# nabw/poroelasticity-linear-solvers

Measured on AMD Instinct MI355X. Metric: Krylov iters/sec + SpMV achieved HBM GB/s, 3-field poroelastic 10M DoF, higher is better.
Workload: dtype f64

## Files before the change

include/pls.h:

```cpp
#ifndef PLS_H
#define PLS_H

#include <stdint.h>

#ifdef __cplusplus
extern "C" {
#endif

#define PLS_ABI_VERSION 1

typedef struct pls_csr {
    int64_t nrows;
    int64_t ncols;
    const int64_t *row_ptr;
    const int32_t *col;
    const double *val;
} pls_csr;

typedef struct pls_handle pls_handle;
typedef struct pls_comm pls_comm;

typedef int (*pls_allgather_fn)(const void *send, int64_t bytes, void *recv, void *user);

typedef struct pls_result {
// ... 89 lines not shown
                              double *c_val);
int pls_hessenberg_eigenvalues(int m, const double *H, int ldh, double *re, double *im);

int pls_export_matrix(pls_handle *h, int which, int64_t *nrows, int64_t *nnz,
                      int64_t *row_ptr, int32_t *col, double *val);
int pls_get_permutation(pls_handle *h, int64_t *perm);

int pls_boomeramg_host_level(const pls_csr *A, const char *options, const char *prefix, int64_t level,
                             int64_t *nlevels, int64_t *n, int64_t *nc, int64_t *p_nnz, int8_t *cf, int64_t *p_rp,
                             int32_t *p_ci, double *p_v);

int pls_sparse_lu_analyze(const pls_csr *A, const char *options, double *stats, int64_t nstats, int32_t *perm,
                          int32_t *front_of, int32_t *parent);

typedef struct pls_anderson pls_anderson;
int pls_anderson_create(int32_t order, int64_t n, pls_anderson **out);
int pls_anderson_next(pls_anderson *a, double *d_gk);
int pls_anderson_destroy(pls_anderson *a);

int pls_bench_spmv(pls_handle *h, const double *d_x, double *d_y, int32_t reps, double *sec_per_launch);
int pls_bench_spmv_single(pls_handle *h, const double *d_x, double *d_y, int32_t reps, double *sec_per_launch);
int pls_spmv_layout(pls_handle *h, int32_t *d16, int64_t *matrix_bytes);
int pls_spmv_layout_single(pls_handle *h, int32_t *d16, int64_t *matrix_bytes);
int pls_bench_copy(int64_t bytes, int32_t reps, int32_t read_only, double *gbs);

#ifdef __cplusplus
}
#endif
#endif
```

poroelasticity-linear-solvers_amd/csrc/capi.cpp:

```cpp
#include <hip/hip_runtime.h>

#include <algorithm>
#include <atomic>
#include <chrono>
#include <numeric>

#include "../../include/pls.h"
#include "runtime.hpp"
#include "amg_host.hpp"
#include "anderson.hpp"
#include "bccols.hpp"
#include "blockpc.hpp"
#include "dist.hpp"
#include "synthetic.hpp"

namespace pls {

static thread_local std::string g_last_error;

static std::string checked_pc_type(const Options &o) {
    std::string pt = o.str("pls.pc_type", "diagonal");
    std::replace(pt.begin(), pt.end(), '_', ' ');
    static const char *ok[] = {"undrained", "undrained 3-way", "diagonal", "diagonal 3-way", "diagonal 3-way-II", "lu"};
    for (auto s : ok)
// ... 21 lines not shown
    std::unique_ptr<KSP> outer;
    AAR aar;
    DBuf<double> vout;
    pls_result res{};
    std::vector<double> history;
    std::unique_ptr<MatOp> Aop;
    Coupling coupling;
    bool coupling_stale = true;

    void parse_params() {
        pc_type = checked_pc_type(opt);
        three_way = (pc_type == "diagonal 3-way" || pc_type == "undrained 3-way");
        solver_type = opt.str("pls.solver_type", "gmres");
        inner_ksp = opt.str("pls.inner_ksp_type", "gmres");
        inner_pc = opt.str("pls.inner_pc_type", "hypre");
        timers.enabled = opt.flag("pls.timers", true);
        ctx.sell_d16 = opt.flag("pls.sell_d16", true);
        ctx.d16_wide_lpr = (int)opt.integer("pls.d16_wide_lpr", 8);
        if (ctx.d16_wide_lpr != 1 && ctx.d16_wide_lpr != 2 && ctx.d16_wide_lpr != 4 && ctx.d16_wide_lpr != 8 &&
            ctx.d16_wide_lpr != 16 && ctx.d16_wide_lpr != 32 && ctx.d16_wide_lpr != 64)
            throw Error("pls.d16_wide_lpr must be a power of two <= 64");
        ctx.d16_unroll = (int)opt.integer("pls.d16_unroll", 4);
        ctx.d16_xcd = (int)opt.integer("pls.d16_xcd", 0);
        ctx.d16_unroll_single = (int)opt.integer("pls.d16_unroll_single", 8);
        if (ctx.d16_unroll_single != 1 && ctx.d16_unroll_single != 2 && ctx.d16_unroll_single != 4 &&
            ctx.d16_unroll_single != 8)
            throw Error("pls.d16_unroll_single must be 1, 2, 4 or 8");
        ctx.halo_overlap = opt.flag("pls.halo_overlap", true);
        ctx.d16_segs = (int)opt.integer("pls.d16_segs", D16_SEG);
        if (ctx.d16_segs != D16_SEG && ctx.d16_segs != D16_SEG_MAX) throw Error("pls.d16_segs must be 4 or 8");
        ctx.d16_sigma = (int)opt.integer("pls.d16_sigma", 1024);
        if (ctx.d16_sigma < 0 || ctx.d16_sigma % 64) throw Error("pls.d16_sigma must be a multiple of 64 (0: off)");
        ctx.d16_sigma_pad = opt.num("pls.d16_sigma_pad", 0.15);
        ctx.d16_sorted_lpr = (int)opt.integer("pls.d16_sorted_lpr", 2);
        ctx.spmv_b3 = opt.flag("pls.spmv_b3", false);
        ctx.spmv_rcm = (int)opt.integer("pls.spmv_rcm", -1);
        ctx.sweep_chain = (int)opt.integer("pls.sweep_chain", -1);
        ctx.sweep_window = (int)opt.integer("pls.sweep_window", -1);
        ctx.ilu_factor_dep = (int)opt.integer("pls.ilu_factor_dep", 1);
        ctx.ilu_view = (int)opt.integer("pls.ilu_view", 0);
        ctx.ilu0_stage_cap = (int)opt.integer("pls.ilu0_stage", -1);
        ctx.ilu_dep_grid = (int)opt.integer("pls.ilu_dep_grid", 0);
        ctx.window_depth = (int)opt.integer("pls.window_depth", 2);
        if (ctx.window_depth != 2 && ctx.window_depth != 3) throw Error("pls.window_depth must be 2 or 3");
        ctx.window_ring = (int)opt.integer("pls.window_ring", -1);
        ctx.window_mixed = (int)opt.integer("pls.window_mixed", -1);
// ... 922 lines not shown
        (void)hipStreamDestroy(st);
    })
}

int pls_spmv_layout(pls_handle *hh, int32_t *d16, int64_t *matrix_bytes) {
    PLS_TRY({
        Handle &H = *reinterpret_cast<Handle *>(hh);
        build_sell(H.A, H.ctx);
        if (d16) *d16 = H.A.sell && H.A.sell->d16 ? 1 : 0;
        if (matrix_bytes) *matrix_bytes = H.A.sell ? H.A.sell->bytes() : 0;
    })
}

int pls_spmv_layout_single(pls_handle *hh, int32_t *d16, int64_t *matrix_bytes) {
    PLS_TRY({
        Handle &H = *reinterpret_cast<Handle *>(hh);
        build_sell(H.A, H.ctx);
        const bool ok = H.A.sell && H.A.sell->d16 && !H.A.sell->b3_nslices;
        if (d16) *d16 = ok ? 1 : 0;
        if (matrix_bytes) *matrix_bytes = ok ? H.A.sell->bytes_low() : 0;
    })
}

}
```

poroelasticity-linear-solvers_amd/csrc/kernels.hip:

```cpp
#include "devutil.hpp"

#include <hipcub/hipcub.hpp>

#include <type_traits>

namespace pls {

__device__ __forceinline__ double wave_reduce(double v) {
#pragma unroll
    for (int o = 32; o > 0; o >>= 1) v += __shfl_xor(v, o);
    return v;
}

#pragma clang fp contract(off)

__device__ __forceinline__ uint64_t mix64(uint64_t z) {
    z += 0x9E3779B97F4A7C15ULL;
    z = (z ^ (z >> 30)) * 0xBF58476D1CE4E5B9ULL;
    z = (z ^ (z >> 27)) * 0x94D049BB133111EBULL;
    return z ^ (z >> 31);
}
__device__ __forceinline__ uint64_t hash3(uint64_t s, uint64_t a, uint64_t b) {
    return mix64(mix64(mix64(s) ^ a) ^ b);
}
// ... 1526 lines not shown
    int32_t last = 0;
    for (int64_t k = 0; k < L; ++k) {
        const int64_t j = k * lpr + sub;
        uint16_t d = 0;
        double v = 0.0;
        if (j < len) {
            const int32_t c = ci[s0 + j];
            v = val[s0 + j];
            const int64_t gap = (int64_t)c - (int64_t)last;
            if (k == 0 || gap > 65535 || gap <= 0) {
                seg[slot * nsegs + nseg++] = c;
            } else {
                d = (uint16_t)gap;
            }
            last = c;
        }
        dl[base + (k >> 3) * 512 + lane * 8 + (k & 7)] = d;
        dv[base + (k >> 1) * 128 + lane * 2 + (k & 1)] = v;
    }
    if (nseg == 0) seg[slot * nsegs + nseg++] = 0;
    for (int j = nseg; j < nsegs; ++j) seg[slot * nsegs + j] = seg[slot * nsegs + nseg - 1];
}

__global__ __launch_bounds__(TPB) void k_first_col(int64_t nrows, const int64_t *rp, const int32_t *ci, int32_t *c0) {
    const int64_t r = (int64_t)blockIdx.x * TPB + threadIdx.x;
    if (r < nrows) c0[r] = rp[r + 1] > rp[r] ? ci[rp[r]] : -1;
}

typedef int32_t d16_i4 __attribute__((ext_vector_type(4)));
typedef uint32_t d16_u4 __attribute__((ext_vector_type(4)));
typedef double d16_d2 __attribute__((ext_vector_type(2)));
typedef float d16_f4 __attribute__((ext_vector_type(4)));

template <class V>
struct d16_values;
template <>
struct d16_values<double> {
    typedef d16_d2 pack;
    static constexpr int PER = 2, UNROLL_MAX = 4;
    static constexpr bool AUX_STORE = true;
    static __device__ __forceinline__ double get(const pack v, int e) { return e ? v.y : v.x; }
};
template <>
struct d16_values<float> {
    typedef d16_f4 pack;
    static constexpr int PER = 4, UNROLL_MAX = 8;
    static constexpr bool AUX_STORE = false;
    static __device__ __forceinline__ double get(const pack v, int e) {
        return (double)(e == 0 ? v.x : e == 1 ? v.y : e == 2 ? v.z : v.w);
    }
};

template <int G2, int TAG, bool HALO, int SEG, int AUX, class V>
__global__ __launch_bounds__(TPB) void k_d16_spmv(int64_t nrows, int64_t nslices, const int64_t *__restrict__ sptr,
                                                  const int64_t *__restrict__ sfirst,
                                                  const int32_t *__restrict__ slpr,
                                                  const uint16_t *__restrict__ dl, const V *__restrict__ dv,
                                                  const int32_t *__restrict__ seg, const double *__restrict__ x,
                                                  double *__restrict__ y, double alpha, double beta,
                                                  const double *__restrict__ z, const double *__restrict__ ghost,
                                                  int32_t nlocal, const int32_t *__restrict__ slist,
                                                  const int32_t *__restrict__ rowmap, double *aux, int d16_xcd) {
    static_assert(SEG == 4 || SEG == 8, "segment bases are one or two int4 per lane");
    static_assert(AUX != D16_AUX_STORE || d16_values<V>::AUX_STORE, "the raw-sum store belongs to the fp64 launch");
    typedef typename d16_values<V>::pack pack;
    constexpr int PER = d16_values<V>::PER, NQ = 8 / PER;
    const int lane = threadIdx.x & 63;
    unsigned blk = blockIdx.x;
    if (d16_xcd) {
        const unsigned per = (gridDim.x + 7) / 8;
        blk = (blockIdx.x % 8) * per + blockIdx.x / 8;
    }
    const int64_t idx = __builtin_amdgcn_readfirstlane((int)(blk * (TPB / 64) + (threadIdx.x >> 6)));
    if (idx >= nslices) return;
    const int64_t sl = slist ? (int64_t)__builtin_amdgcn_readfirstlane(slist[idx]) : idx;
    const int64_t base = sptr[sl];
    const int64_t L = (sptr[sl + 1] - base) >> 6;
    const int lpr = slpr[sl];
    const int64_t r0 = sfirst[sl], r1 = sfirst[sl + 1];
    const int64_t row = r0 + lane / lpr;
    const d16_i4 sb = __builtin_nontemporal_load(reinterpret_cast<const d16_i4 *>(seg) + (sl * 64 + lane) * (SEG / 4));
    d16_i4 sb2 = sb;
    if (SEG == 8) sb2 = __builtin_nontemporal_load(reinterpret_cast<const d16_i4 *>(seg) + (sl * 64 + lane) * 2 + 1);
    const d16_u4 *dp = reinterpret_cast<const d16_u4 *>(dl + base) + lane;
    const pack *vp = reinterpret_cast<const pack *>(dv + base) + lane;
    int32_t col = 0;
    int si = 0;
    double acc = 0.0;
    if (AUX == D16_AUX_INIT && lpr == 1 && row < r1) acc = aux[row];
    const int64_t ng = L >> 3;
    for (int64_t g0 = 0; g0 < ng; g0 += G2) {
        d16_u4 d[G2];
        pack v[G2][NQ];
#pragma unroll
        for (int u = 0; u < G2; ++u) {
            const int64_t g = g0 + u < ng ? g0 + u : ng - 1;
            d[u] = __builtin_nontemporal_load(dp + g * 64);
#pragma unroll
            for (int q = 0; q < NQ; ++q) v[u][q] = __builtin_nontemporal_load(vp + (g * NQ + q) * 64);
        }
#pragma unroll
        for (int u = 0; u < G2; ++u) {
            if (g0 + u >= ng) break;
            const uint32_t w[4] = {d[u].x, d[u].y, d[u].z, d[u].w};
#pragma unroll
            for (int e = 0; e < 8; ++e) {
                const int32_t dd = (int32_t)((w[e >> 1] >> ((e & 1) * 16)) & 0xffffu);
                int32_t b = si == 0 ? sb.x : si == 1 ? sb.y : si == 2 ? sb.z : sb.w;
                if (SEG == 8 && si >= 4) b = si == 4 ? sb2.x : si == 5 ? sb2.y : si == 6 ? sb2.z : sb2.w;
                col = dd == 0 ? b : col + dd;
                si += dd == 0 ? 1 : 0;
                const double a = d16_values<V>::get(v[u][e / PER], e % PER);
                if (HALO) {
                    const bool loc = col < nlocal;
                    const double xv = loc ? x[(uint32_t)col] : ghost[(uint32_t)(col - nlocal)];
                    acc += a * xv;
                } else {
                    acc += a * x[(uint32_t)col];
                }
            }
// ... 11 lines not shown
        y[yr] = r;
    }
}

void launch_d16_slice_len(int64_t nslices, const int64_t *sfirst, const int32_t *slpr, const int64_t *rp,
                          int64_t nrows, int64_t *slen, hipStream_t st, const int32_t *rowmap, const int64_t *rstart) {
    k_d16_slice_len<<<grid_for((nslices + 1) * 64, TPB), TPB, 0, st>>>(nslices, sfirst, slpr, rp, nrows, slen, rowmap,
                                                                       rstart);
}
void launch_d16_count(int64_t nslices, const int64_t *sfirst, const int32_t *slpr, const int64_t *rp,
                      const int32_t *ci, int64_t nrows, int32_t *maxseg, hipStream_t st, const int32_t *rowmap,
                      const int64_t *rstart) {
    if (nslices > 0)
        k_d16_count<<<grid_for(nslices * 64, TPB), TPB, 0, st>>>(nslices, sfirst, slpr, rp, ci, nrows, maxseg, rowmap,
                                                                 rstart);
}
void launch_d16_fill(int64_t nslices, const int64_t *sfirst, const int32_t *slpr, const int64_t *rp,
                     const int32_t *ci, const double *val, int64_t nrows, const int64_t *sptr, uint16_t *dl,
                     double *dv, int32_t *seg, int nsegs, hipStream_t st, const int32_t *rowmap,
                     const int64_t *rstart) {
    if (nslices > 0)
        k_d16_fill<<<grid_for(nslices * 64, TPB), TPB, 0, st>>>(nslices, sfirst, slpr, rp, ci, val, nrows, sptr, dl,
                                                                dv, seg, nsegs, rowmap, rstart);
}
__global__ __launch_bounds__(TPB) void k_coupling_rows(int64_t n, int64_t ns, const int64_t *rp, const int32_t *ci,
                                                       const double *val, const int64_t *mrp, const int32_t *mci,
                                                       const double *mval, const uint8_t *reuse, int64_t *rstart,
                                                       int32_t *differs) {
    const int64_t r = (int64_t)blockIdx.x * TPB + threadIdx.x;
    if (r >= n) return;
    const int64_t s = rp[r], e = rp[r + 1];
    if (r < ns) {
        rstart[r] = s;
        return;
    }
    int64_t lo = s, hi = e;
    while (lo < hi) {
        const int64_t mid = (lo + hi) >> 1;
        if (ci[mid] < ns) lo = mid + 1;
        else hi = mid;
    }
    const int64_t m0 = mrp[r - ns], cnt = lo - s;
    bool same = mrp[r - ns + 1] - m0 == cnt;
    for (int64_t k = 0; k < cnt && same; ++k)
        same = ci[s + k] == mci[m0 + k] && __double_as_longlong(val[s + k]) == __double_as_longlong(mval[m0 + k]);
    if (!same) *differs = 1;
// ... 9 lines not shown
    if (nrows > 0) k_first_col<<<grid_for(nrows, TPB), TPB, 0, st>>>(nrows, rp, ci, c0);
}
template <class V>
struct D16Call {
    unsigned g;
    size_t shm;
    hipStream_t st;
    int64_t nrows, ns;
    D16Streams L;
    const V *dv;
    const double *x;
    double *y;
    double alpha, beta;
    const double *z, *ghost;
    int32_t nl;
    const int32_t *slist, *rm;
    double *aux;
    int d16_xcd;
};
template <int G2, int TAG, bool HALO, int SEG, int AUX, class V>
static void d16_go(const D16Call<V> &a) {
    k_d16_spmv<G2, TAG, HALO, SEG, AUX, V><<<a.g, TPB, a.shm, a.st>>>(a.nrows, a.ns, a.L.sptr, a.L.sfirst, a.L.slpr,
                                                                      a.L.dl, a.dv, a.L.seg, a.x, a.y, a.alpha, a.beta,
                                                                      a.z, a.ghost, a.nl, a.slist, a.rm, a.aux, a.d16_xcd);
}
template <int G2, int SEG, class V>
static void d16_dispatch(const D16Call<V> &a, int tag, int aux_mode) {
    if constexpr (d16_values<V>::AUX_STORE)
        if (aux_mode == D16_AUX_STORE) return d16_go<G2, 0, false, SEG, D16_AUX_STORE>(a);
    if (aux_mode != D16_AUX_NONE) return d16_go<G2, 1, false, SEG, D16_AUX_INIT>(a);
    if (a.ghost) {
        if (tag) d16_go<G2, 1, true, SEG, D16_AUX_NONE>(a);
        else d16_go<G2, 0, true, SEG, D16_AUX_NONE>(a);
    } else {
        if (tag) d16_go<G2, 1, false, SEG, D16_AUX_NONE>(a);
        else d16_go<G2, 0, false, SEG, D16_AUX_NONE>(a);
    }
}
template <int SEG, class V>
static void d16_unrolled(int unroll, const D16Call<V> &a, int tag, int aux_mode) {
    switch (unroll) {
        case 1: d16_dispatch<1, SEG>(a, tag, aux_mode); break;
        case 2: d16_dispatch<2, SEG>(a, tag, aux_mode); break;
        case 4: d16_dispatch<4, SEG>(a, tag, aux_mode); break;
        default: d16_dispatch<d16_values<V>::UNROLL_MAX, SEG>(a, tag, aux_mode); break;
    }
}
// ... 865 lines not shown
```

poroelasticity-linear-solvers_amd/csrc/kernels.hpp:

```cpp
#pragma once
#include <hip/hip_runtime.h>
#include <cstdint>

namespace pls {

struct SynthDev {
    int32_t dim;
    uint64_t seed;
    double delta;
    int64_t n[3];
    int64_t off[3];
    int32_t cnt[6];
    const int32_t *offs[6];
    int64_t rlo[3], rlen[3], rloff[3], nrows;
};
void launch_synth_count(const SynthDev &S, int64_t *row_len, hipStream_t st);
void launch_synth_fill(const SynthDev &S, int variant, const int64_t *row_ptr, int32_t *col,
                       double *val, hipStream_t st);
void launch_synth_rhs(const SynthDev &S, uint64_t seed, double *b, hipStream_t st);

void exclusive_scan_i64(const int64_t *in, int64_t *out, int64_t n, void *tmp, size_t tmp_bytes,
                        hipStream_t st);
size_t exclusive_scan_tmp_bytes(int64_t n);

// ... 146 lines not shown
void launch_iluk_scatter(int64_t n, const int64_t *srp, const int32_t *sci, const double *sval, const int64_t *drp,
                         const int32_t *dci, double *dval, int32_t *fail, hipStream_t st);

int64_t sell_nslices(int64_t nrows);
void launch_sell_slice_len(int64_t nrows, const int64_t *rp, int64_t *slen , hipStream_t st);
void launch_sell_fill(int64_t nrows, const int64_t *rp, const int32_t *ci, const double *val, const int64_t *sptr,
                      int32_t *scol, double *sval, hipStream_t st);
void launch_sell_spmv(int64_t nrows, const int64_t *sptr, const int32_t *scol, const double *sval, const double *x,
                      double *y, double alpha, double beta, const double *z, int tag, const double *ghost,
                      int64_t nlocal, hipStream_t st);
constexpr int D16_SEG = 4;
constexpr int D16_SEG_MAX = 8;
void launch_d16_slice_len(int64_t nslices, const int64_t *sfirst, const int32_t *slpr, const int64_t *rp,
                          int64_t nrows, int64_t *slen , hipStream_t st,
                          const int32_t *rowmap = nullptr ,
                          const int64_t *rstart = nullptr);
void launch_d16_count(int64_t nslices, const int64_t *sfirst, const int32_t *slpr, const int64_t *rp,
                      const int32_t *ci, int64_t nrows, int32_t *maxseg, hipStream_t st,
                      const int32_t *rowmap = nullptr, const int64_t *rstart = nullptr);
void launch_d16_fill(int64_t nslices, const int64_t *sfirst, const int32_t *slpr, const int64_t *rp,
                     const int32_t *ci, const double *val, int64_t nrows, const int64_t *sptr, uint16_t *dl,
                     double *dv, int32_t *seg, int nsegs , hipStream_t st,
                     const int32_t *rowmap = nullptr, const int64_t *rstart = nullptr);
void launch_coupling_rows(int64_t n, int64_t ns, const int64_t *rp, const int32_t *ci, const double *val,
                          const int64_t *mrp, const int32_t *mci, const double *mval, const uint8_t *reuse,
                          int64_t *rstart, int32_t *differs, hipStream_t st);
constexpr int D16_AUX_NONE = 0, D16_AUX_STORE = 1, D16_AUX_INIT = 2;
void launch_first_col(int64_t nrows, const int64_t *rp, const int32_t *ci, int32_t *c0, hipStream_t st);
struct D16Streams {
    const int64_t *sptr, *sfirst;
    const int32_t *slpr;
    const uint16_t *dl;
    const int32_t *seg;
    int nsegs;
};
void launch_d16_spmv(int64_t nrows, int64_t nslices, const D16Streams &L, const double *dv, const double *x, double *y,
                     double alpha, double beta, const double *z, int tag, const double *ghost, int64_t nlocal,
                     int unroll ,
                     int d16_xcd ,
                     hipStream_t st,
                     const int32_t *slist = nullptr ,
                     const int32_t *rowmap = nullptr ,
                     size_t lds_reserve = 0 ,
                     int aux_mode = D16_AUX_NONE, double *aux = nullptr );
void launch_d16_round_values(int64_t stored, const double *dv, float *dv32, int32_t *overflow, hipStream_t st);
void launch_d16_spmv(int64_t nrows, int64_t nslices, const D16Streams &L, const float *dv32, const double *x, double *y,
                     double alpha, double beta, const double *z, int tag, const double *ghost, int64_t nlocal,
                     int unroll, int d16_xcd, hipStream_t st, const int32_t *slist = nullptr,
                     const int32_t *rowmap = nullptr, size_t lds_reserve = 0, const double *aux_init = nullptr);
void launch_triple_flags(int64_t n, const int64_t *rp, const int32_t *ci, uint8_t *flag, hipStream_t st);
int b3_lanes_per_triple();
void launch_b3_fill(int64_t nslices, int64_t ntrip, const int64_t *bptr, const int32_t *tmap, const int64_t *rp,
                    const int32_t *ci, const double *val, int32_t *bcol, double *bval, hipStream_t st);
void launch_b3_spmv(int64_t nslices, int64_t ntrip, const int64_t *bptr, const int32_t *tmap, const int32_t *bcol,
                    const double *bval, const double *x, double *y, double alpha, double beta, const double *z,
                    int tag, hipStream_t st);
void launch_row_has_ghost(int64_t nrows, const int64_t *rp, const int32_t *ci, int64_t nlocal, uint8_t *flag,
// ... 164 lines not shown
```

poroelasticity-linear-solvers_amd/csrc/runtime.cpp:

```cpp
#include "runtime.hpp"

#include <sys/mman.h>

#include <algorithm>
#include <thread>
#include <functional>
#include <numeric>
#include <cmath>
#include <cstdio>
#include <cstring>
#include <sstream>

namespace pls {

void *huge_alloc(size_t bytes) {
    const size_t len = (bytes + HUGE_ALLOC_MIN - 1) & ~(HUGE_ALLOC_MIN - 1);
    void *p = mmap(nullptr, len, PROT_READ | PROT_WRITE, MAP_PRIVATE | MAP_ANONYMOUS, -1, 0);
    if (p == MAP_FAILED) throw std::bad_alloc();
    (void)madvise(p, len, MADV_HUGEPAGE);
    return p;
}
void huge_free(void *p, size_t bytes) {
    if (p) (void)munmap(p, (bytes + HUGE_ALLOC_MIN - 1) & ~(HUGE_ALLOC_MIN - 1));
}
// ... 392 lines not shown
    c.spmv_rcm = keep;
    if (!Mp.sell || !Mp.sell->d16 || Mp.sell->b3_nslices) return false;
    DevSELL &S = *Mp.sell;
    std::vector<int32_t> rm(n);
    if (S.nrows_mapped) {
        HIPCHK(hipMemcpyAsync(rm.data(), S.rowmap.p, sizeof(int32_t) * n, hipMemcpyDeviceToHost, c.st));
        c.sync();
        for (auto &r : rm) r = ord[r];
    } else {
        rm = ord;
    }
    S.rowmap.alloc(n);
    S.nrows_mapped = n;
    HIPCHK(hipMemcpyAsync(S.rowmap.p, rm.data(), sizeof(int32_t) * n, hipMemcpyHostToDevice, c.st));
    S.xperm.alloc(n);
    HIPCHK(hipMemcpyAsync(S.xperm.p, ord.data(), sizeof(int32_t) * n, hipMemcpyHostToDevice, c.st));
    S.nperm = n;
    if (c.rcm_x.n < (size_t)n) c.rcm_x.alloc(n);
    c.sync();
    M.sell = std::move(Mp.sell);
    return true;
}

static bool d16_from_plan(const DevCSR &M, DevSELL &S, const std::vector<int64_t> &sf, const std::vector<int32_t> &lp,
                          const std::vector<int32_t> &rm, const int64_t *rstart, Ctx &c) {
    const int64_t ns = (int64_t)lp.size();
    S.sfirst.alloc(ns + 1);
    S.slpr.alloc(std::max<int64_t>(ns, 1));
    HIPCHK(hipMemcpyAsync(S.sfirst.p, sf.data(), sizeof(int64_t) * (ns + 1), hipMemcpyHostToDevice, c.st));
    HIPCHK(hipMemcpyAsync(S.slpr.p, lp.data(), sizeof(int32_t) * ns, hipMemcpyHostToDevice, c.st));
    if (!rm.empty()) {
        S.rowmap.alloc(rm.size());
        S.nrows_mapped = (int64_t)rm.size();
        HIPCHK(hipMemcpyAsync(S.rowmap.p, rm.data(), sizeof(int32_t) * rm.size(), hipMemcpyHostToDevice, c.st));
    }
    const int32_t *rmap = rm.empty() ? nullptr : S.rowmap.p;
    DBuf<int32_t> mx(1);
    HIPCHK(hipMemsetAsync(mx.p, 0, sizeof(int32_t), c.st));
    launch_d16_count(ns, S.sfirst.p, S.slpr.p, M.rp.p, M.ci.p, M.nrows, mx.p, c.st, rmap, rstart);
    int32_t h = 0;
    HIPCHK(hipMemcpyAsync(&h, mx.p, sizeof(int32_t), hipMemcpyDeviceToHost, c.st));
    c.sync();
    S.d16 = h <= D16_SEG_MAX;
    S.nsegs = (h <= D16_SEG && c.d16_segs <= D16_SEG) ? D16_SEG : D16_SEG_MAX;
    if (!S.d16) return false;
    S.nslices = ns;
    for (int32_t l : lp) S.wide_slices += (l > 1);
    DBuf<int64_t> slen(ns + 1);
    launch_d16_slice_len(ns, S.sfirst.p, S.slpr.p, M.rp.p, M.nrows, slen.p, c.st, rmap, rstart);
    S.sptr.alloc(ns + 1);
    c.ensure_scan(ns);
    exclusive_scan_i64(slen.p, S.sptr.p, ns, c.scan_tmp.p, c.scan_tmp_bytes, c.st);
    HIPCHK(hipMemcpyAsync(&S.stored, S.sptr.p + ns, sizeof(int64_t), hipMemcpyDeviceToHost, c.st));
    c.sync();
    S.val.alloc(std::max<int64_t>(S.stored, 2));
    S.dl.alloc(std::max<int64_t>(S.stored, 8));
    S.seg.alloc(ns * 64 * S.nsegs);
    launch_d16_fill(ns, S.sfirst.p, S.slpr.p, M.rp.p, M.ci.p, M.val.p, M.nrows, S.sptr.p, S.dl.p, S.val.p, S.seg.p,
                    S.nsegs, c.st, rmap, rstart);
    HIPCHK(hipGetLastError());
    c.sync();
    return true;
}

void build_sell(DevCSR &M, Ctx &c) {
    if (M.sell || M.nrows == 0) return;
    if (c.spmv_rcm != 0 && c.sell_d16 && !c.spmv_b3 && !M.halo && M.nrows == M.ncols && M.nrows >= 16384) {
        bool pads = c.spmv_rcm == 1;
        if (!pads && M.rcm_auto) {
            std::vector<int64_t> sf;
            std::vector<int32_t> lp, rm;
            d16_plan(M, sf, lp, rm, c);
            pads = !rm.empty();
        }
        if (pads && build_sell_rcm(M, c)) return;
    }
    auto S = std::make_unique<DevSELL>();
    if (c.sell_d16 && M.nnz > 0) {
        std::vector<int64_t> sf;
        std::vector<int32_t> lp, rm, singles;
        const bool b3 = build_b3(M, *S, singles, c);
        d16_plan(M, sf, lp, rm, c, b3 ? &singles : nullptr);
        const int64_t ns = (int64_t)lp.size();
        if (ns == 0) {
// ... 683 lines not shown
            row.push_back({lj, L.v[k]});
        }
        std::sort(row.begin(), row.end(), [](const auto &a, const auto &b) { return a.first < b.first; });
        for (auto &e : row) {
            T.ci.push_back(e.first);
            T.v.push_back(e.second);
        }
        T.rp.push_back((int64_t)T.ci.size());
    }
    upload(T, M, c);
    M.ncols = T.ncols;
    M.halo = H;
    M.sell.reset();
    build_sell(M, c);
    c.sync();
}

std::unique_ptr<Ctx> layout_ctx(const Ctx &c) {
    auto self = std::make_unique<Ctx>();
    self->sell_d16 = c.sell_d16;
    self->d16_wide_lpr = c.d16_wide_lpr;
    self->d16_unroll = c.d16_unroll;
    self->d16_xcd = c.d16_xcd;
    self->d16_unroll_single = c.d16_unroll_single;
    self->d16_segs = c.d16_segs;
    self->d16_sigma = c.d16_sigma;
    self->d16_sigma_pad = c.d16_sigma_pad;
    self->d16_sorted_lpr = c.d16_sorted_lpr;
    self->spmv_b3 = c.spmv_b3;
    self->spmv_rcm = c.spmv_rcm;
    self->sweep_chain = c.sweep_chain;
    self->sweep_window = c.sweep_window;
    self->window_depth = c.window_depth;
    self->window_ring = c.window_ring;
    self->window_mixed = c.window_mixed;
    self->window_kpw = c.window_kpw;
    self->amg_csr_below = c.amg_csr_below;
    return self;
}

struct PCRedundant : PC {
    std::unique_ptr<Ctx> self;
    DevCSR Gm;
    std::unique_ptr<PC> inner;
    int64_t nloc = 0, maxloc = 0, N = 0;
    DBuf<int64_t> src, mine;
// ... 382 lines not shown
```

poroelasticity-linear-solvers_amd/csrc/runtime.hpp:

```cpp
#pragma once
#include <hip/hip_runtime.h>

#include <cmath>
#include <cstdint>
#include <map>
#include <functional>
#include <memory>
#include <stdexcept>
#include <string>
#include <vector>

#include "comm.hpp"
#include "kernels.hpp"

namespace pls {

struct Error : std::runtime_error {
    explicit Error(const std::string &m) : std::runtime_error(m) {}
};

#define HIPCHK(x)                                                                                   \
    do {                                                                                            \
        hipError_t e_ = (x);                                                                        \
        if (e_ != hipSuccess)                                                                       \
// ... 20 lines not shown
        n = count;
        if (count) HIPCHK(hipMalloc((void **)&p, sizeof(T) * count));
    }
    void release() {
        if (p) (void)hipFree(p);
        p = nullptr;
        n = 0;
    }
    T *get() const { return p; }
};

struct Ctx {
    hipStream_t st = nullptr;
    Comm *comm = nullptr;
    DBuf<double> partial;
    int64_t partial_n = 0;
    int64_t hscal_n = 0;
    DBuf<double> dscal;
    double *hscal = nullptr;
    bool sell_d16 = true;
    int d16_wide_lpr = 8;
    int d16_unroll = 4;
    int d16_xcd = 0;
    int d16_unroll_single = 8;
    int d16_segs = D16_SEG;
    int d16_sigma = 1024;
    double d16_sigma_pad = 0.15;
    int d16_sorted_lpr = 2;
    bool spmv_b3 = false;
    int spmv_rcm = -1;
    int sweep_chain = -1;
    int sweep_window = -1;
    int ilu_factor_dep = 1;
    int ilu_view = 0;
    int ilu0_stage_cap = -1;
    int ilu_dep_grid = 0;
    int window_depth = 2;
    int window_ring = -1;
    int window_kpw = 0;
    int window_mixed = -1;
    int sweep_swin = 0;
    double amg_csr_below = 16.0;
    bool halo_overlap = true;
    hipStream_t st_comm = nullptr;
    hipEvent_t ev_x = nullptr, ev_halo = nullptr;
    DBuf<char> scan_tmp;
// ... 2 lines not shown
    std::vector<int64_t> rank_rows;
    Ctx();
    ~Ctx();
    void sync() { HIPCHK(hipStreamSynchronize(st)); }
    void ensure_scan(int64_t n);
    void ensure_partial(int64_t n, int64_t cols);
    double *partials(int64_t n, int64_t cols);
    double *host_scalars(int64_t count);
    bool debug_bounds = false, debug_no_grow = false, debug_unguarded = false;
    static constexpr int64_t CANARY = 1 << 16;
    void set_debug(bool bounds, int64_t cap, bool no_grow, bool unguarded);
    void check_bounds();
    double dot(int64_t n, const double *x, const double *y);
    double norm2(int64_t n, const double *x);
};

struct DevSELL {
    int64_t nslices = 0, stored = 0;
    bool d16 = false;
    DBuf<int64_t> sptr;
    DBuf<int32_t> col;
    DBuf<double> val;
    DBuf<uint16_t> dl;
    DBuf<int32_t> seg, slpr;
    DBuf<int64_t> sfirst;
    int64_t wide_slices = 0;
    DBuf<int32_t> rowmap;
    int64_t nrows_mapped = 0;
    int64_t b3_nslices = 0, b3_ntrip = 0, b3_stored = 0;
    DBuf<int64_t> b3ptr;
    DBuf<int32_t> b3map, b3col;
    DBuf<double> b3val;
    int nsegs = D16_SEG;
    DBuf<int32_t> s_in, s_halo;
    int64_t n_in = 0, n_halo = 0;
    int64_t nperm = 0;
    DBuf<int32_t> xperm;
    DBuf<float> val32;
    D16Streams streams() const { return {sptr.p, sfirst.p, slpr.p, dl.p, seg.p, nsegs}; }
    bool has_low() const { return d16 && !b3_nslices && val32.p != nullptr; }
    int64_t low_stream_bytes() const { return has_low() ? stored * 4 : 0; }
    int64_t bytes_low() const { return bytes() - stored * 4; }
    int64_t bytes() const {
        return (d16 ? stored * 10 + nslices * (64 * 4 * nsegs + 20) + 8 + nrows_mapped * 4
                    : stored * 12 + (nslices + 1) * 8) +
               b3_stored * 28 + b3_ntrip * 4 + (b3_nslices + 1) * 8 + nperm * 20;
    }
};

struct Halo {
    int64_t nlocal = 0, nghost = 0, nsend = 0;
    std::vector<int64_t> l2g;
    DBuf<int32_t> send_idx;
    DBuf<double> sendbuf, ghost;
    std::vector<int64_t> scnt, soff, rcnt, roff;
};

struct DevCSR {
    int64_t nrows = 0, ncols = 0, nnz = 0;
    std::shared_ptr<Halo> halo;
    DBuf<int64_t> rp;
    DBuf<int32_t> ci;
    DBuf<double> val;
    int64_t max_row = 0;
    std::unique_ptr<DevSELL> sell;
    int tag = 0;
    bool rcm_auto = true;
// ... 365 lines not shown
```

poroelasticity-linear-solvers_amd/lib/_native.py:

```python
from __future__ import annotations

import ctypes as C
import os

import numpy as np

_PKG = os.path.dirname(os.path.dirname(os.path.abspath(__file__)))
LIB_PATH = os.path.join(_PKG, "libpls.so")

_lib = None


class pls_csr(C.Structure):
    _fields_ = [("nrows", C.c_int64), ("ncols", C.c_int64), ("row_ptr", C.c_void_p),
                ("col", C.c_void_p), ("val", C.c_void_p)]


class pls_result(C.Structure):
    _fields_ = [("its", C.c_int32), ("reason", C.c_int32), ("rnorm", C.c_double),
                ("pc_applies", C.c_int32), ("history_len", C.c_int32)]


class pls_timings(C.Structure):
    _fields_ = [("pc_total", C.c_double), ("pc_solid", C.c_double), ("pc_fluid", C.c_double),
# ... 1 lines not shown
                ("spmv_total", C.c_double), ("spmv_calls", C.c_int64)]


class pls_synth_spec(C.Structure):
    _fields_ = [("dim", C.c_int32), ("N", C.c_int32), ("seed", C.c_uint64), ("delta", C.c_double)]


EXPORTS = [
    "pls_abi_version", "pls_last_error", "pls_device_count", "pls_set_device", "pls_create",
    "pls_create_synthetic", "pls_setup", "pls_set_option", "pls_create_solver", "pls_destroy",
    "pls_get_sizes", "pls_pc_apply", "pls_solve", "pls_matmult", "pls_solve_device",
    "pls_pc_apply_device", "pls_matmult_device", "pls_synthetic_rhs_device", "pls_device_alloc",
    "pls_device_free", "pls_memcpy_h2d", "pls_memcpy_d2h", "pls_get_result", "pls_get_history",
    "pls_get_timings", "pls_reset_timings", "pls_export_matrix", "pls_get_permutation",
    "pls_bench_spmv", "pls_rccl_unique_id", "pls_comm_create_rccl", "pls_comm_create_callback",
    "pls_comm_destroy", "pls_create_synthetic_dist", "pls_spmv_layout", "pls_update_matrices",
    "pls_bench_copy", "pls_create_dist", "pls_bench_global_sum", "pls_anderson_create",
    "pls_anderson_next", "pls_anderson_destroy", "pls_boomeramg_host_level", "pls_sparse_lu_analyze",
    "pls_get_ksp_stats", "pls_get_gmres_orthog_stats", "pls_get_chebyshev_bounds",
    "pls_hessenberg_eigenvalues", "pls_get_reuse_stats", "pls_get_ilu_fill",
    "pls_get_gmres_basis_stats", "pls_get_ksp_guess_stats", "pls_get_ksp_guess_info",
    "pls_matmult_single", "pls_matmult_single_device", "pls_spmv_layout_single", "pls_bench_spmv_single",
    "pls_get_gmres_operator_stats", "pls_get_reuse_rows", "pls_get_asm_stats", "pls_get_asm_rows",
    "pls_get_bc_columns_stats", "pls_get_bc_columns_matrix",
]

ALLGATHER_FN = C.CFUNCTYPE(C.c_int, C.c_void_p, C.c_int64, C.c_void_p, C.c_void_p)


def lib():
    global _lib
    if _lib is not None:
        return _lib
    if not os.path.exists(LIB_PATH):
        raise RuntimeError(f"libpls.so not found at {LIB_PATH}; build it with "
                           f"`python -c 'import __graft_entry__ as g; g.build()'`")
    L = C.CDLL(LIB_PATH)
    vp, i64, i32 = C.c_void_p, C.c_int64, C.c_int32
    L.pls_last_error.restype = C.c_char_p
    L.pls_device_count.argtypes = [C.POINTER(C.c_int)]
    L.pls_set_device.argtypes = [C.c_int]
    L.pls_create.argtypes = [C.POINTER(pls_csr), C.POINTER(pls_csr), C.POINTER(pls_csr),
                             vp, i64, vp, i64, vp, i64, vp, i64, C.c_char_p, C.POINTER(vp)]
    L.pls_create_synthetic.argtypes = [C.POINTER(pls_synth_spec), C.c_char_p, C.POINTER(vp)]
    for f in ("pls_setup", "pls_create_solver", "pls_destroy", "pls_reset_timings"):
        getattr(L, f).argtypes = [vp]
    L.pls_set_option.argtypes = [vp, C.c_char_p, C.c_char_p]
# ... 10 lines not shown
    L.pls_memcpy_h2d.argtypes = [vp, vp, i64]
    L.pls_memcpy_d2h.argtypes = [vp, vp, i64]
    L.pls_get_result.argtypes = [vp, C.POINTER(pls_result)]
    L.pls_get_history.argtypes = [vp, vp, i32]
    L.pls_get_timings.argtypes = [vp, C.POINTER(pls_timings)]
    L.pls_get_ksp_stats.argtypes = [vp, C.c_char_p, vp]
    L.pls_get_gmres_orthog_stats.argtypes = [vp, C.c_char_p, vp]
    L.pls_get_gmres_basis_stats.argtypes = [vp, C.c_char_p, vp]
    L.pls_get_gmres_operator_stats.argtypes = [vp, C.c_char_p, vp]
    L.pls_get_reuse_rows.argtypes = [vp, vp]
    L.pls_matmult_single.argtypes = [vp, vp, vp]
    L.pls_matmult_single_device.argtypes = [vp, vp, vp]
    L.pls_bench_spmv_single.argtypes = [vp, vp, vp, i32, C.POINTER(C.c_double)]
    L.pls_spmv_layout_single.argtypes = [vp, C.POINTER(i32), C.POINTER(i64)]
    L.pls_get_ksp_guess_stats.argtypes = [vp, C.c_char_p, vp, C.POINTER(C.c_double)]
    L.pls_get_ksp_guess_info.argtypes = [vp, C.c_char_p, C.POINTER(i64), C.POINTER(C.c_double)]
    L.pls_get_chebyshev_bounds.argtypes = [vp, C.c_char_p, vp]
    L.pls_get_ilu_fill.argtypes = [vp, C.c_char_p, vp]
    L.pls_get_asm_stats.argtypes = [vp, C.c_char_p, vp]
    L.pls_get_asm_rows.argtypes = [vp, C.c_char_p, vp, vp]
    L.pls_get_bc_columns_stats.argtypes = [vp, C.c_char_p, vp]
    L.pls_get_bc_columns_matrix.argtypes = [vp, C.c_char_p, vp, vp, vp, vp]
    L.pls_get_reuse_stats.argtypes = [vp, vp]
    L.pls_hessenberg_eigenvalues.argtypes = [C.c_int, vp, C.c_int, vp, vp]
    L.pls_export_matrix.argtypes = [vp, C.c_int, C.POINTER(i64), C.POINTER(i64), vp, vp, vp]
    L.pls_get_permutation.argtypes = [vp, vp]
    L.pls_bench_spmv.argtypes = [vp, vp, vp, i32, C.POINTER(C.c_double)]
    L.pls_rccl_unique_id.argtypes = [C.c_char_p]
    L.pls_comm_create_rccl.argtypes = [C.c_char_p, C.c_int, C.c_int, C.POINTER(vp)]
    L.pls_comm_create_callback.argtypes = [C.c_int, C.c_int, ALLGATHER_FN, vp, C.POINTER(vp)]
    L.pls_comm_destroy.argtypes = [vp]
    L.pls_update_matrices.argtypes = [vp, C.POINTER(pls_csr), C.POINTER(pls_csr), C.POINTER(pls_csr)]
    L.pls_bench_copy.argtypes = [i64, i32, i32, C.POINTER(C.c_double)]
    L.pls_spmv_layout.argtypes = [vp, C.POINTER(i32), C.POINTER(i64)]
    L.pls_create_synthetic_dist.argtypes = [C.POINTER(pls_synth_spec), C.c_char_p, vp, C.POINTER(vp)]
    L.pls_bench_global_sum.argtypes = [vp, i32, i32, C.POINTER(C.c_double)]
    L.pls_anderson_create.argtypes = [i32, i64, C.POINTER(vp)]
    L.pls_anderson_next.argtypes = [vp, vp]
    L.pls_anderson_destroy.argtypes = [vp]
    L.pls_boomeramg_host_level.argtypes = [C.POINTER(pls_csr), C.c_char_p, C.c_char_p, i64, C.POINTER(i64),
                                           C.POINTER(i64), C.POINTER(i64), C.POINTER(i64), vp, vp, vp, vp]
    L.pls_sparse_lu_analyze.argtypes = [C.POINTER(pls_csr), C.c_char_p, vp, i64, vp, vp, vp]
    L.pls_create_dist.argtypes = [C.POINTER(pls_csr), C.POINTER(pls_csr), C.POINTER(pls_csr), i64,
                                  vp, i64, vp, i64, vp, i64, vp, i64, C.c_char_p, vp, C.POINTER(vp)]
    _lib = L
    return L
# ... 79 lines not shown
```

poroelasticity-linear-solvers_amd/lib/handle.py:

```python
from __future__ import annotations

import ctypes as C

import numpy as np

from . import _native as N


def params_to_options(parameters: dict) -> dict:
    keymap = {
        "solver type": "pls.solver_type", "solver atol": "pls.solver_atol", "solver rtol": "pls.solver_rtol",
        "solver maxiter": "pls.solver_maxiter", "solver monitor": "pls.solver_monitor",
        "pc type": "pls.pc_type", "inner ksp type": "pls.inner_ksp_type", "inner pc type": "pls.inner_pc_type",
        "inner rtol": "pls.inner_rtol", "inner atol": "pls.inner_atol", "inner maxiter": "pls.inner_maxiter",
        "inner monitor": "pls.inner_monitor", "inner accel order": "pls.inner_accel_order",
        "AAR order": "pls.aar_order", "AAR p": "pls.aar_p", "AAR omega": "pls.aar_omega", "AAR beta": "pls.aar_beta",
    }
    out = {}
    for k, v in parameters.items():
        if k in keymap:
            if isinstance(v, bool):
                v = "1" if v else "0"
            out[keymap[k]] = str(v).replace(" ", "_")
    return out
# ... 261 lines not shown

    def bc_columns_stats(self, prefix):
        s = np.zeros(5, dtype=np.int64)
        N.check(N.lib().pls_get_bc_columns_stats(self.ptr, prefix.encode(), N.ptr(s)))
        return tuple(int(v) for v in s)

    def bc_columns_matrix(self, prefix):
        sizes = {"s_": self.ns, "f_": self.nf, "p_": self.np, "diff_": self.np, "fp_": self.nf + self.np,
                 "fp_fieldsplit_0_": self.np, "fp_fieldsplit_1_": self.nf}
        if prefix not in sizes:
            raise ValueError(f"Handle.bc_columns_matrix: no inner solver with prefix {prefix!r}")
        s = self.bc_columns_stats(prefix)
        rows = np.zeros(max(s[1], 1), dtype=np.int32)
        rp = np.zeros(sizes[prefix] + 1, dtype=np.int64)
        ci = np.zeros(max(s[2], 1), dtype=np.int32)
        v = np.zeros(max(s[2], 1), dtype=np.float64)
        N.check(N.lib().pls_get_bc_columns_matrix(self.ptr, prefix.encode(), N.ptr(rows), N.ptr(rp), N.ptr(ci),
                                                  N.ptr(v)))
        return rows[:s[1]], rp, ci[:s[2]], v[:s[2]]

    def reuse_stats(self):
        s = np.zeros(3, dtype=np.int64)
        N.check(N.lib().pls_get_reuse_stats(self.ptr, N.ptr(s)))
        return tuple(int(v) for v in s)

    def reuse_rows(self):
        m = np.zeros(self.n, dtype=np.uint8)
        N.check(N.lib().pls_get_reuse_rows(self.ptr, N.ptr(m)))
        return m

    def reset_timings(self):
        N.check(N.lib().pls_reset_timings(self.ptr))

    def export_matrix(self, which=0):
        import scipy.sparse as sp
        nr, nnz = C.c_int64(), C.c_int64()
        N.check(N.lib().pls_export_matrix(self.ptr, which, C.byref(nr), C.byref(nnz), None, None, None))
        rp = np.zeros(nr.value + 1, dtype=np.int64)
        ci = np.zeros(nnz.value, dtype=np.int32)
        v = np.zeros(nnz.value, dtype=np.float64)
        N.check(N.lib().pls_export_matrix(self.ptr, which, C.byref(nr), C.byref(nnz), N.ptr(rp), N.ptr(ci), N.ptr(v)))
        return sp.csr_matrix((v, ci, rp), shape=(nr.value, nr.value))

    def permutation(self):
        p = np.zeros(self.n, dtype=np.int64)
        N.check(N.lib().pls_get_permutation(self.ptr, N.ptr(p)))
# ... 43 lines not shown
```

Before: 186.9.

## Deduplicate identical per-lane column-delta streams in d16 SELL slices

At setup, each 64-row slice of the d16 SELL layout is hashed per lane, and lanes whose 16-bit column-delta streams are identical are grouped into classes. Only one copy per class is stored, and the SpMV kernel reads deltas through a per-lane class index with a compacted stride. The aim is to cut HBM bytes for column indices on a structured poroelastic matrix where rows share stencil patterns. In exchange there is extra setup work, a per-lane class lookup plus a max-reduction in the kernel, and more divergent delta loads. The commit also raises the launch-bounds occupancy hint for one kernel variant and adds a stats query.

```diff
diff --git a/include/pls.h b/include/pls.h
--- a/include/pls.h
+++ b/include/pls.h
@@ -135,6 +135,7 @@
 int pls_bench_spmv_single(pls_handle *h, const double *d_x, double *d_y, int32_t reps, double *sec_per_launch);
 int pls_spmv_layout(pls_handle *h, int32_t *d16, int64_t *matrix_bytes);
 int pls_spmv_layout_single(pls_handle *h, int32_t *d16, int64_t *matrix_bytes);
+int pls_get_d16_share(pls_handle *h, int32_t which, int64_t stats[5]);
 int pls_bench_copy(int64_t bytes, int32_t reps, int32_t read_only, double *gbs);
 
 #ifdef __cplusplus
diff --git a/poroelasticity-linear-solvers_amd/csrc/capi.cpp b/poroelasticity-linear-solvers_amd/csrc/capi.cpp
--- a/poroelasticity-linear-solvers_amd/csrc/capi.cpp
+++ b/poroelasticity-linear-solvers_amd/csrc/capi.cpp
@@ -67,6 +67,9 @@
             throw Error("pls.d16_wide_lpr must be a power of two <= 64");
         ctx.d16_unroll = (int)opt.integer("pls.d16_unroll", 4);
         ctx.d16_xcd = (int)opt.integer("pls.d16_xcd", 0);
+        ctx.d16_share = (int)opt.integer("pls.d16_share", -1);
+        if (ctx.d16_share < -1 || ctx.d16_share > 1) throw Error("pls.d16_share must be -1, 0 or 1");
+        ctx.d16_share_min_bytes = opt.integer("pls.d16_share_min_bytes", 268435456);
         ctx.d16_unroll_single = (int)opt.integer("pls.d16_unroll_single", 8);
         if (ctx.d16_unroll_single != 1 && ctx.d16_unroll_single != 2 && ctx.d16_unroll_single != 4 &&
             ctx.d16_unroll_single != 8)
@@ -1035,4 +1038,20 @@
     })
 }
 
-}
+int pls_get_d16_share(pls_handle *hh, int32_t which, int64_t *stats) {
+    PLS_TRY({
+        Handle &H = *reinterpret_cast<Handle *>(hh);
+        if (!stats) throw Error("pls_get_d16_share: null argument");
+        if (which != 0 && which != 1) throw Error("pls_get_d16_share: which must be 0 (A) or 1 (the reduced outer layout)");
+        if (which == 0) build_sell(H.A, H.ctx);
+        const DevSELL *S = which == 0 ? H.A.sell.get() : H.coupling.eligible ? &H.coupling.reduced : nullptr;
+        const bool d16 = S && S->d16;
+        stats[0] = d16 && S->cls.p ? 1 : 0;
+        stats[1] = d16 ? S->nslices : 0;
+        stats[2] = d16 ? S->shared_slices : 0;
+        stats[3] = d16 ? S->dstored : 0;
+        stats[4] = H.ctx.d16_share_built;
+    })
+}
+
+}
diff --git a/poroelasticity-linear-solvers_amd/csrc/kernels.hip b/poroelasticity-linear-solvers_amd/csrc/kernels.hip
--- a/poroelasticity-linear-solvers_amd/csrc/kernels.hip
+++ b/poroelasticity-linear-solvers_amd/csrc/kernels.hip
@@ -1572,13 +1572,78 @@
     for (int j = nseg; j < nsegs; ++j) seg[slot * nsegs + j] = seg[slot * nsegs + nseg - 1];
 }
 
+typedef uint32_t d16_u4 __attribute__((ext_vector_type(4)));
+
+__device__ __forceinline__ int d16_lowest_equal(uint64_t key, int lane) {
+    int rep = lane;
+    for (int j = 63; j >= 0; --j) {
+        const uint64_t kj = __shfl(key, j);
+        if (kj == key) rep = j;
+    }
+    return rep;
+}
+
+__global__ __launch_bounds__(TPB) void k_d16_share_classes(int64_t nslices, const int64_t *__restrict__ sptr,
+                                                           const uint16_t *__restrict__ dl, uint8_t *cls,
+                                                           int64_t *cnt, int64_t *nshared) {
+    const int64_t sl = ((int64_t)blockIdx.x * TPB + threadIdx.x) >> 6;
+    const int lane = threadIdx.x & 63;
+    if (sl > nslices) return;
+    if (sl == nslices) { if (lane == 0) cnt[nslices] = 0; return; }
+    const int64_t base = sptr[sl];
+    const int64_t L = (sptr[sl + 1] - base) >> 6;
+    const int64_t ng = L >> 3;
+    const d16_u4 *dp = reinterpret_cast<const d16_u4 *>(dl + base);
+    uint64_t h = 0xcbf29ce484222325ull;
+    for (int64_t g = 0; g < ng; ++g) {
+        const d16_u4 d = dp[g * 64 + lane];
+        h = (h ^ (((uint64_t)d.y << 32) | d.x)) * 0x9e3779b97f4a7c15ull;
+        h ^= h >> 29;
+        h = (h ^ (((uint64_t)d.w << 32) | d.z)) * 0xbf58476d1ce4e5b9ull;
+        h ^= h >> 32;
+    }
+    const int rep = d16_lowest_equal(h, lane);
+    bool same = true;
+    if (rep != lane)
+        for (int64_t g = 0; g < ng && same; ++g) {
+            const d16_u4 a = dp[g * 64 + lane], b = dp[g * 64 + rep];
+            same = a.x == b.x && a.y == b.y && a.z == b.z && a.w == b.w;
+        }
+    const bool ok = !__any(!same);
+    const uint64_t reps = ok ? __ballot(rep == lane) : ~0ull;
+    const int c = ok ? __popcll(reps & ((1ull << rep) - 1ull)) : lane;
+    const int C = __popcll(reps);
+    cls[sl * 64 + lane] = (uint8_t)c;
+    if (lane == 0) {
+        cnt[sl] = C * L;
+        if (C < 64) atomicAdd(reinterpret_cast<unsigned long long *>(nshared), 1ull);
+    }
+}
+
+__global__ __launch_bounds__(TPB) void k_d16_share_fill(int64_t nslices, const int64_t *__restrict__ sptr,
+                                                        const int64_t *__restrict__ dptr,
+                                                        const uint8_t *__restrict__ cls,
+                                                        const uint16_t *__restrict__ dl, uint16_t *dls) {
+    const int64_t sl = ((int64_t)blockIdx.x * TPB + threadIdx.x) >> 6;
+    const int lane = threadIdx.x & 63;
+    if (sl >= nslices) return;
+    const int64_t base = sptr[sl];
+    const int64_t ng = (sptr[sl + 1] - base) >> 9;
+    const int c = cls[sl * 64 + lane];
+    const bool first = d16_lowest_equal((uint64_t)c, lane) == lane;
+    const int C = __popcll(__ballot(first));
+    if (!first) return;
+    const d16_u4 *src = reinterpret_cast<const d16_u4 *>(dl + base) + lane;
+    d16_u4 *dst = reinterpret_cast<d16_u4 *>(dls + dptr[sl]) + c;
+    for (int64_t g = 0; g < ng; ++g) dst[g * C] = src[g * 64];
+}
+
 __global__ __launch_bounds__(TPB) void k_first_col(int64_t nrows, const int64_t *rp, const int32_t *ci, int32_t *c0) {
     const int64_t r = (int64_t)blockIdx.x * TPB + threadIdx.x;
     if (r < nrows) c0[r] = rp[r + 1] > rp[r] ? ci[rp[r]] : -1;
 }
 
 typedef int32_t d16_i4 __attribute__((ext_vector_type(4)));
-typedef uint32_t d16_u4 __attribute__((ext_vector_type(4)));
 typedef double d16_d2 __attribute__((ext_vector_type(2)));
 typedef float d16_f4 __attribute__((ext_vector_type(4)));
 
@@ -1602,7 +1667,7 @@
 };
 
 template <int G2, int TAG, bool HALO, int SEG, int AUX, class V>
-__global__ __launch_bounds__(TPB) void k_d16_spmv(int64_t nrows, int64_t nslices, const int64_t *__restrict__ sptr,
+__global__ __launch_bounds__(TPB, (G2 == 8 && SEG == 4 && HALO) ? 4 : 1) void k_d16_spmv(int64_t nrows, int64_t nslices, const int64_t *__restrict__ sptr,
                                                   const int64_t *__restrict__ sfirst,
                                                   const int32_t *__restrict__ slpr,
                                                   const uint16_t *__restrict__ dl, const V *__restrict__ dv,
@@ -1610,7 +1675,9 @@
                                                   double *__restrict__ y, double alpha, double beta,
                                                   const double *__restrict__ z, const double *__restrict__ ghost,
                                                   int32_t nlocal, const int32_t *__restrict__ slist,
-                                                  const int32_t *__restrict__ rowmap, double *aux, int d16_xcd) {
+                                                  const int32_t *__restrict__ rowmap, double *aux, int d16_xcd,
+                                                  const int64_t *__restrict__ dptr,
+                                                  const uint8_t *__restrict__ cls) {
     static_assert(SEG == 4 || SEG == 8, "segment bases are one or two int4 per lane");
     static_assert(AUX != D16_AUX_STORE || d16_values<V>::AUX_STORE, "the raw-sum store belongs to the fp64 launch");
     typedef typename d16_values<V>::pack pack;
@@ -1632,7 +1699,20 @@
     const d16_i4 sb = __builtin_nontemporal_load(reinterpret_cast<const d16_i4 *>(seg) + (sl * 64 + lane) * (SEG / 4));
     d16_i4 sb2 = sb;
     if (SEG == 8) sb2 = __builtin_nontemporal_load(reinterpret_cast<const d16_i4 *>(seg) + (sl * 64 + lane) * 2 + 1);
-    const d16_u4 *dp = reinterpret_cast<const d16_u4 *>(dl + base) + lane;
+    int64_t dbase = base, gs = 64;
+    int dlane = lane;
+    if (cls) {
+        dlane = cls[sl * 64 + lane];
+        int C = dlane;
+#pragma unroll
+        for (int o = 32; o > 0; o >>= 1) {
+            const int t = __shfl_xor(C, o);
+            C = t > C ? t : C;
+        }
+        gs = __builtin_amdgcn_readfirstlane(C) + 1;
+        dbase = dptr[sl];
+    }
+    const d16_u4 *dp = reinterpret_cast<const d16_u4 *>(dl + dbase) + dlane;
     const pack *vp = reinterpret_cast<const pack *>(dv + base) + lane;
     int32_t col = 0;
     int si = 0;
@@ -1645,7 +1725,7 @@
 #pragma unroll
         for (int u = 0; u < G2; ++u) {
             const int64_t g = g0 + u < ng ? g0 + u : ng - 1;
-            d[u] = __builtin_nontemporal_load(dp + g * 64);
+            d[u] = __builtin_nontemporal_load(dp + g * gs);
 #pragma unroll
             for (int q = 0; q < NQ; ++q) v[u][q] = __builtin_nontemporal_load(vp + (g * NQ + q) * 64);
         }
@@ -1703,6 +1783,15 @@
     if (nslices > 0)
         k_d16_fill<<<grid_for(nslices * 64, TPB), TPB, 0, st>>>(nslices, sfirst, slpr, rp, ci, val, nrows, sptr, dl,
                                                                 dv, seg, nsegs, rowmap, rstart);
+}
+void launch_d16_share_classes(int64_t nslices, const int64_t *sptr, const uint16_t *dl, uint8_t *cls, int64_t *cnt,
+                              int64_t *nshared, hipStream_t st) {
+    k_d16_share_classes<<<grid_for((nslices + 1) * 64, TPB), TPB, 0, st>>>(nslices, sptr, dl, cls, cnt, nshared);
+}
+void launch_d16_share_fill(int64_t nslices, const int64_t *sptr, const int64_t *dptr, const uint8_t *cls,
+                           const uint16_t *dl, uint16_t *dls, hipStream_t st) {
+    if (nslices > 0)
+        k_d16_share_fill<<<grid_for(nslices * 64, TPB), TPB, 0, st>>>(nslices, sptr, dptr, cls, dl, dls);
 }
 __global__ __launch_bounds__(TPB) void k_coupling_rows(int64_t n, int64_t ns, const int64_t *rp, const int32_t *ci,
                                                        const double *val, const int64_t *mrp, const int32_t *mci,
@@ -1758,7 +1847,8 @@
 static void d16_go(const D16Call<V> &a) {
     k_d16_spmv<G2, TAG, HALO, SEG, AUX, V><<<a.g, TPB, a.shm, a.st>>>(a.nrows, a.ns, a.L.sptr, a.L.sfirst, a.L.slpr,
                                                                       a.L.dl, a.dv, a.L.seg, a.x, a.y, a.alpha, a.beta,
-                                                                      a.z, a.ghost, a.nl, a.slist, a.rm, a.aux, a.d16_xcd);
+                                                                      a.z, a.ghost, a.nl, a.slist, a.rm, a.aux, a.d16_xcd,
+                                                                      a.L.dptr, a.L.cls);
 }
 template <int G2, int SEG, class V>
 static void d16_dispatch(const D16Call<V> &a, int tag, int aux_mode) {
diff --git a/poroelasticity-linear-solvers_amd/csrc/kernels.hpp b/poroelasticity-linear-solvers_amd/csrc/kernels.hpp
--- a/poroelasticity-linear-solvers_amd/csrc/kernels.hpp
+++ b/poroelasticity-linear-solvers_amd/csrc/kernels.hpp
@@ -192,6 +192,10 @@
                      const int32_t *ci, const double *val, int64_t nrows, const int64_t *sptr, uint16_t *dl,
                      double *dv, int32_t *seg, int nsegs , hipStream_t st,
                      const int32_t *rowmap = nullptr, const int64_t *rstart = nullptr);
+void launch_d16_share_classes(int64_t nslices, const int64_t *sptr, const uint16_t *dl, uint8_t *cls, int64_t *cnt,
+                              int64_t *nshared, hipStream_t st);
+void launch_d16_share_fill(int64_t nslices, const int64_t *sptr, const int64_t *dptr, const uint8_t *cls,
+                           const uint16_t *dl, uint16_t *dls, hipStream_t st);
 void launch_coupling_rows(int64_t n, int64_t ns, const int64_t *rp, const int32_t *ci, const double *val,
                           const int64_t *mrp, const int32_t *mci, const double *mval, const uint8_t *reuse,
                           int64_t *rstart, int32_t *differs, hipStream_t st);
@@ -203,6 +207,8 @@
     const uint16_t *dl;
     const int32_t *seg;
     int nsegs;
+    const int64_t *dptr = nullptr;
+    const uint8_t *cls = nullptr;
 };
 void launch_d16_spmv(int64_t nrows, int64_t nslices, const D16Streams &L, const double *dv, const double *x, double *y,
                      double alpha, double beta, const double *z, int tag, const double *ghost, int64_t nlocal,
diff --git a/poroelasticity-linear-solvers_amd/csrc/runtime.cpp b/poroelasticity-linear-solvers_amd/csrc/runtime.cpp
--- a/poroelasticity-linear-solvers_amd/csrc/runtime.cpp
+++ b/poroelasticity-linear-solvers_amd/csrc/runtime.cpp
@@ -438,6 +438,33 @@
     return true;
 }
 
+static void d16_share(DevSELL &S, Ctx &c) {
+    const int64_t ns = S.nslices;
+    if (c.d16_share == 0 || ns == 0 || S.stored == 0) return;
+    if (c.d16_share < 0 && S.bytes() <= c.d16_share_min_bytes) return;
+    DBuf<uint8_t> cls(ns * 64);
+    DBuf<int64_t> cnt(ns + 1), dptr(ns + 1), nshared(1);
+    HIPCHK(hipMemsetAsync(nshared.p, 0, sizeof(int64_t), c.st));
+    launch_d16_share_classes(ns, S.sptr.p, S.dl.p, cls.p, cnt.p, nshared.p, c.st);
+    c.ensure_scan(ns);
+    exclusive_scan_i64(cnt.p, dptr.p, ns, c.scan_tmp.p, c.scan_tmp_bytes, c.st);
+    int64_t total = 0, shared = 0;
+    HIPCHK(hipMemcpyAsync(&total, dptr.p + ns, sizeof(int64_t), hipMemcpyDeviceToHost, c.st));
+    HIPCHK(hipMemcpyAsync(&shared, nshared.p, sizeof(int64_t), hipMemcpyDeviceToHost, c.st));
+    c.sync();
+    if (c.d16_share < 0 && total * 2 + ns * 72 + 8 >= S.stored * 2) return;
+    DBuf<uint16_t> dls(std::max<int64_t>(total, 8));
+    launch_d16_share_fill(ns, S.sptr.p, dptr.p, cls.p, S.dl.p, dls.p, c.st);
+    HIPCHK(hipGetLastError());
+    c.sync();
+    S.dl = std::move(dls);
+    S.dptr = std::move(dptr);
+    S.cls = std::move(cls);
+    S.dstored = total;
+    S.shared_slices = shared;
+    ++c.d16_share_built;
+}
+
 static bool d16_from_plan(const DevCSR &M, DevSELL &S, const std::vector<int64_t> &sf, const std::vector<int32_t> &lp,
                           const std::vector<int32_t> &rm, const int64_t *rstart, Ctx &c) {
     const int64_t ns = (int64_t)lp.size();
@@ -476,6 +503,8 @@
                     S.nsegs, c.st, rmap, rstart);
     HIPCHK(hipGetLastError());
     c.sync();
+    S.dstored = S.stored;
+    d16_share(S, c);
     return true;
 }
 
@@ -1205,6 +1234,8 @@
     self->d16_wide_lpr = c.d16_wide_lpr;
     self->d16_unroll = c.d16_unroll;
     self->d16_xcd = c.d16_xcd;
+    self->d16_share = c.d16_share;
+    self->d16_share_min_bytes = c.d16_share_min_bytes;
     self->d16_unroll_single = c.d16_unroll_single;
     self->d16_segs = c.d16_segs;
     self->d16_sigma = c.d16_sigma;
diff --git a/poroelasticity-linear-solvers_amd/csrc/runtime.hpp b/poroelasticity-linear-solvers_amd/csrc/runtime.hpp
--- a/poroelasticity-linear-solvers_amd/csrc/runtime.hpp
+++ b/poroelasticity-linear-solvers_amd/csrc/runtime.hpp
@@ -66,6 +66,9 @@
     int d16_wide_lpr = 8;
     int d16_unroll = 4;
     int d16_xcd = 0;
+    int d16_share = -1;
+    int64_t d16_share_min_bytes = 268435456;
+    int64_t d16_share_built = 0;
     int d16_unroll_single = 8;
     int d16_segs = D16_SEG;
     int d16_sigma = 1024;
@@ -114,6 +117,9 @@
     DBuf<int32_t> col;
     DBuf<double> val;
     DBuf<uint16_t> dl;
+    DBuf<int64_t> dptr;
+    DBuf<uint8_t> cls;
+    int64_t dstored = 0, shared_slices = 0;
     DBuf<int32_t> seg, slpr;
     DBuf<int64_t> sfirst;
     int64_t wide_slices = 0;
@@ -129,12 +135,13 @@
     int64_t nperm = 0;
     DBuf<int32_t> xperm;
     DBuf<float> val32;
-    D16Streams streams() const { return {sptr.p, sfirst.p, slpr.p, dl.p, seg.p, nsegs}; }
+    D16Streams streams() const { return {sptr.p, sfirst.p, slpr.p, dl.p, seg.p, nsegs, dptr.p, cls.p}; }
     bool has_low() const { return d16 && !b3_nslices && val32.p != nullptr; }
     int64_t low_stream_bytes() const { return has_low() ? stored * 4 : 0; }
     int64_t bytes_low() const { return bytes() - stored * 4; }
     int64_t bytes() const {
-        return (d16 ? stored * 10 + nslices * (64 * 4 * nsegs + 20) + 8 + nrows_mapped * 4
+        return (d16 ? stored * 8 + dstored * 2 + (cls.p ? nslices * 72 + 8 : 0) + nslices * (64 * 4 * nsegs + 20) + 8 +
+                          nrows_mapped * 4
                     : stored * 12 + (nslices + 1) * 8) +
                b3_stored * 28 + b3_ntrip * 4 + (b3_nslices + 1) * 8 + nperm * 20;
     }
diff --git a/poroelasticity-linear-solvers_amd/lib/_native.py b/poroelasticity-linear-solvers_amd/lib/_native.py
--- a/poroelasticity-linear-solvers_amd/lib/_native.py
+++ b/poroelasticity-linear-solvers_amd/lib/_native.py
@@ -47,7 +47,7 @@
     "pls_get_gmres_basis_stats", "pls_get_ksp_guess_stats", "pls_get_ksp_guess_info",
     "pls_matmult_single", "pls_matmult_single_device", "pls_spmv_layout_single", "pls_bench_spmv_single",
     "pls_get_gmres_operator_stats", "pls_get_reuse_rows", "pls_get_asm_stats", "pls_get_asm_rows",
-    "pls_get_bc_columns_stats", "pls_get_bc_columns_matrix",
+    "pls_get_bc_columns_stats", "pls_get_bc_columns_matrix", "pls_get_d16_share",
 ]
 
 ALLGATHER_FN = C.CFUNCTYPE(C.c_int, C.c_void_p, C.c_int64, C.c_void_p, C.c_void_p)
@@ -104,6 +104,7 @@
     L.pls_get_bc_columns_stats.argtypes = [vp, C.c_char_p, vp]
     L.pls_get_bc_columns_matrix.argtypes = [vp, C.c_char_p, vp, vp, vp, vp]
     L.pls_get_reuse_stats.argtypes = [vp, vp]
+    L.pls_get_d16_share.argtypes = [vp, i32, vp]
     L.pls_hessenberg_eigenvalues.argtypes = [C.c_int, vp, C.c_int, vp, vp]
     L.pls_export_matrix.argtypes = [vp, C.c_int, C.POINTER(i64), C.POINTER(i64), vp, vp, vp]
     L.pls_get_permutation.argtypes = [vp, vp]
diff --git a/poroelasticity-linear-solvers_amd/lib/handle.py b/poroelasticity-linear-solvers_amd/lib/handle.py
--- a/poroelasticity-linear-solvers_amd/lib/handle.py
+++ b/poroelasticity-linear-solvers_amd/lib/handle.py
@@ -307,6 +307,11 @@
     def reuse_stats(self):
         s = np.zeros(3, dtype=np.int64)
         N.check(N.lib().pls_get_reuse_stats(self.ptr, N.ptr(s)))
+        return tuple(int(v) for v in s)
+
+    def d16_share(self, which=0):
+        s = np.zeros(5, dtype=np.int64)
+        N.check(N.lib().pls_get_d16_share(self.ptr, int(which), N.ptr(s)))
         return tuple(int(v) for v in s)
 
     def reuse_rows(self):
```

Measured after the change: 204.1, median of 6. +9.2%, better.
